# vmanam0451/distributed-path-tracer

Hardware: AMD Instinct MI355X
Metric: Msamples/sec, Cornell box 1920x1080, 256 spp per frame, 8 bounces (camera paths traced per second) (higher is better)
Workload: dtype f32

## Files before the change

### distributed-path-tracer_amd/__init__.py

```python
import atexit
import ctypes as C
import os
import re
import weakref

import numpy as np

_HERE = os.path.dirname(os.path.abspath(__file__))
LIB_PATH = os.environ.get("PTX_LIB") or os.path.join(_HERE, "libptx_hip.so")
HEADER_PATH = os.path.join(os.path.dirname(_HERE), "include", "ptx.h")

OK, ERR_INVALID, ERR_IO, ERR_PARSE, ERR_NO_CAMERA, ERR_NO_DEVICE, ERR_HIP, ERR_UNSUPPORTED = range(8)
NO_SUN_LIGHT = 0xFFFFFFFF

(ARR_MODEL_XFORM, ARR_MODEL_AABB, ARR_MODEL_SURF, ARR_SURF_RANGE, ARR_MESH_AABB, ARR_VERTICES, ARR_TRIANGLES,
 ARR_MATERIALS, ARR_KD_NODES, ARR_KD_REFS, ARR_CAMERA, ARR_SUN, ARR_MODEL_NAMES, ARR_TEXTURES, ARR_TEXELS, ARR_SURF_TEX, ARR_TEXELS_F32,
 ARR_LIGHT_TRIS, ARR_LIGHT_CDF, ARR_LIGHT_GEOM, ARR_TRI_ISECT, ARR_RES_NODES, ARR_RES_REFS, ARR_RES_TRIS, ARR_LDS_ROOT,
 ARR_RES_PLAN, ARR_ENV_ROW_CDF, ARR_ENV_CELL_CDF, ARR_PUNCTUAL, ARR_PUNCTUAL_CDF, ARR_LENS) = range(31)
LDS_LEAF_ORDER_BIT = 0x80000000


class PtxError(RuntimeError):
    def __init__(self, code, msg):
        super().__init__(f"ptx error {code}: {msg}")
        self.code = code


class WorkItem(C.Structure):
    _fields_ = [("mesh_name", C.c_char_p), ("primitives", C.POINTER(C.c_int32)), ("n_primitives", C.c_uint32)]


class LoadOpts(C.Structure):
    _fields_ = [("camera_index", C.c_uint32), ("sun_light_index", C.c_uint32), ("filter_primitives", C.c_uint32),
                ("n_work", C.c_uint32), ("work", C.POINTER(WorkItem))]


class WorkerEvent(C.Structure):
    _fields_ = [("num_workers", C.c_int32), ("n_work_meshes", C.c_uint32), ("worker_id", C.c_char * 64),
                ("scene_root", C.c_char * 256), ("scene_bucket", C.c_char * 128)]


class SceneDesc(C.Structure):
    _fields_ = [("n_models", C.c_uint32), ("model_xform", C.c_void_p), ("model_surf", C.c_void_p),
                ("n_surfaces", C.c_uint32), ("surf_range", C.c_void_p), ("vertices", C.c_void_p),
                ("triangles", C.c_void_p), ("materials", C.c_void_p), ("camera", C.c_void_p), ("sun", C.c_void_p)]


class Camera(C.Structure):
    _fields_ = [("origin", C.c_float * 3), ("basis", C.c_float * 9), ("yfov", C.c_float), ("lens_radius", C.c_float),
                ("focus_distance", C.c_float), ("blades", C.c_uint32), ("blade_rotation", C.c_float)]


# ... 416 lines not shown
                return -1

        fn = MASK_EXCHANGE_FN(thunk)
        n = int(mask.numel()) if hasattr(mask, "numel") else int(mask.size)
        _check(lib().ptx_ctx_set_mask_exchange(self.h, fn, None, _ptr(mask), n))
        self._mask_exchange = (fn, mask)

    def mask_exchange_stats(self):
        calls, ms = C.c_uint64(), C.c_double()
        _check(lib().ptx_ctx_get_mask_exchange_stats(self.h, C.byref(calls), C.byref(ms)))
        return {"calls": calls.value, "wall_ms": ms.value}

    def close(self):
        if getattr(self, "h", None):
            lib().ptx_ctx_destroy(self.h)
            self.h = None
            self._mask_exchange = None

    def __del__(self):
        try:
            self.close()
        except Exception:
            pass


_ARR_DTYPE = {ARR_MODEL_XFORM: (np.float32, 12), ARR_MODEL_AABB: (np.float32, 6), ARR_MODEL_SURF: (np.int32, 2),
              ARR_SURF_RANGE: (np.int32, 8), ARR_MESH_AABB: (np.float32, 6), ARR_VERTICES: (np.float32, 11),
              ARR_TRIANGLES: (np.uint32, 3), ARR_MATERIALS: (np.float32, 11), ARR_KD_NODES: (np.uint32, 2),
              ARR_KD_REFS: (np.uint32, 1), ARR_CAMERA: (np.float32, 1), ARR_SUN: (np.float32, 1),
              ARR_TEXTURES: (np.uint32, 4), ARR_TEXELS: (np.uint8, 1), ARR_SURF_TEX: (np.int32, 7), ARR_TEXELS_F32: (np.float32, 1),
              ARR_LIGHT_TRIS: (np.uint32, 2), ARR_LIGHT_CDF: (np.float32, 1), ARR_LIGHT_GEOM: (np.float32, 4),
              ARR_TRI_ISECT: (np.uint32, 12), ARR_RES_NODES: (np.uint32, 2), ARR_RES_REFS: (np.uint32, 1), ARR_RES_TRIS: (np.uint32, 12),
              ARR_LDS_ROOT: (np.uint32, 1), ARR_RES_PLAN: (np.uint32, 1), ARR_ENV_ROW_CDF: (np.float32, 1), ARR_ENV_CELL_CDF: (np.float32, 1),
              ARR_PUNCTUAL: (np.float32, 16), ARR_PUNCTUAL_CDF: (np.float32, 1), ARR_LENS: (np.float32, 2)}


class Scene:

    def __init__(self, handle, ctx):
        self.h = handle
        self.ctx = ctx
        _live.add(self)

    @classmethod
    def load_gltf(cls, ctx, path, camera_index=0, sun_light_index=0, work=None):
        h = C.c_void_p()
        opts = LoadOpts(camera_index, sun_light_index, 0, 0, None)
        keep = []
        if work is not None:
            items = (WorkItem * max(len(work), 1))()
            for k, (name, prims) in enumerate(work.items()):
                arr = (C.c_int32 * max(len(prims), 1))(*prims)
                keep.append(arr)
                items[k] = WorkItem(name.encode(), arr, len(prims))
            opts = LoadOpts(camera_index, sun_light_index, 1, len(work), items)
        _check(lib().ptx_scene_load_gltf(ctx.h if ctx else None, os.fsencode(path), C.byref(opts), C.byref(h)))
        return cls(h, ctx)

    @classmethod
    def load_event(cls, ctx, event_json, local_scene_root):
        h, cfg, ev = C.c_void_p(), RenderCfg(), WorkerEvent()
        _check(lib().ptx_worker_event_load(ctx.h if ctx else None, os.fsencode(event_json), os.fsencode(local_scene_root),
                                           C.byref(h), C.byref(cfg), C.byref(ev)))
        info = dict(num_workers=ev.num_workers, n_work_meshes=ev.n_work_meshes, worker_id=ev.worker_id.decode(),
                    scene_root=ev.scene_root.decode(), scene_bucket=ev.scene_bucket.decode())
        return cls(h, ctx), cfg, info

# ... 413 lines not shown
```

### distributed-path-tracer_amd/csrc/api_internal.hpp

```cpp
#pragma once
#include <hip/hip_runtime.h>

#include <algorithm>
#include <atomic>
#include <cstdint>
#include <cstdio>
#include <cstdlib>
#include <cstring>
#include <mutex>
#include <string>
#include <vector>

#include "../../include/ptx.h"
#include "kernels.hpp"

#pragma GCC visibility push(hidden)

using namespace ptx;

int set_err(int code, const std::string& m);
#define HIP_TRY(expr)                                                                                           \
	do {                                                                                                        \
		hipError_t e_ = (expr);                                                                                 \
		if (e_ != hipSuccess) return set_err(PTX_ERR_HIP, std::string(#expr) + ": " + hipGetErrorString(e_));   \
// ... 31 lines not shown
	DevBuf round_ws;
	DevBuf denoise;
	DevBuf adaptive, adaptive_state, adaptive_stage;
	hipEvent_t adaptive_ev[2] = {nullptr, nullptr};
	struct MaskExchange {
		ptx_mask_exchange_fn fn = nullptr;
		void* user = nullptr;
		uint8_t* mask = nullptr;
		size_t bytes = 0;
		uint64_t calls = 0;
		double wall_ms = 0;
	} mask_exchange;
	struct WfSet {
		DevBuf qent, pair_hit, seg, first, mask, ctl, spill, stream_buf, flow;
		uint32_t* flow_host = nullptr;
	} wf;
	std::vector<hipEvent_t> events;
	bool timing_on = false;
	std::vector<hipEvent_t> step_events;
	ptx_kernel_timing timing{};
	uint32_t list_key[9] = {0, 0, 0, 0, 0, 0, 0, 0, 0};
	uint32_t list_len = 0;
};

struct ptx_scene {
	ptx_ctx* ctx = nullptr;
	FlatScene host;
	DevBuf d_models, d_surfaces, d_materials, d_nodes, d_refs, d_tris, d_shade, d_tex, d_texels, d_lut, d_spaces, d_model_space, d_wf_order;
	DevBuf d_res_nodes, d_res_refs, d_res_tris, d_texels_f, d_hot;
	DevScene dev{};
	double lds_area_share = 0;
	double wf_pairs_per_ray = 0;
	bool leaf_ordered = true;
	int lds_leaf_order = -1;
	size_t lds_budget = 0;
	int mode = MODE_GLOBAL;
	size_t lds_bytes = 0;
	struct LightList {
		bool built = false, on_device = false;
		std::vector<uint32_t> tris;
		std::vector<float> cdf, geom;
		std::vector<int32_t> surf_first;
		float area = 0;
	} lights;
	std::mutex lights_mu;
	DevBuf d_light_tris, d_light_cdf, d_light_geom, d_light_first;
	struct EnvTable {
		bool built = false, on_device = false;
		uint32_t w = 0, h = 0;
		std::vector<float> row_cdf, cell_cdf;
	} env_table;
	DevBuf d_env_row, d_env_cell;
	struct Punctual {
		bool on_device = false;
		std::vector<float> recs, cdf;
	} punctual;
	DevBuf d_punctual, d_punctual_cdf;
	DevBuf d_lens;
};

const ptx_scene::LightList* build_lights(ptx_scene* sc);
const ptx_scene::EnvTable* build_env_table(ptx_scene* sc);
void srgb_thresholds(float thr[256]);
int adaptive_decide_locked(ptx_ctx* c, uint32_t w, uint32_t h, const float4* d_a, const float4* d_b, float threshold, uint8_t* d_done, uint32_t* d_pixels, uint32_t& n_active,
                           double* select_ms);
int adaptive_decide_sharded_locked(ptx_ctx* c, uint32_t w, uint32_t h, const AdaptiveShard& shard, bool mask_on_device, const float4* d_a, const float4* d_b, float threshold,
// ... 114 lines not shown
```

### distributed-path-tracer_amd/csrc/api_render.cpp

```cpp
#include <cmath>

#include "api_internal.hpp"

namespace {

int32_t max_surfaces_per_model(const ptx_scene* sc) {
	int32_t m = 0;
	for (const ModelRec& mr : sc->host.models) m = std::max(m, mr.n_surfaces);
	return m;
}

constexpr uint64_t kWfPoolPairs = 1024ull << 20;
constexpr uint64_t kWfBatchPairs = 256ull << 20;
constexpr uint32_t kWfFlowWords = 64, kWfFlowRays = 58 , kWfFlowPeak = 60, kWfFlowOverflow = 63, kWfMaxRound = 56;
bool wf_eligible(const ptx_scene* sc) {
	const size_t n_surf = sc->host.surfaces.size();
	if (n_surf == 0 || n_surf > (size_t)kWfMaxSurfaces) return false;
	if (sc->mode == MODE_LDS || !sc->dev.tri_isect) return false;
	return sc->leaf_ordered && sc->dev.geom_bytes <= 0xFFFFFFFFull;
}
int pipeline_choice(const ptx_scene* sc) {
	if (!wf_eligible(sc)) return 0;
	if (const char* e = getenv("PTX_WAVEFRONT")) return e[0] == '1' ? 1 : 0;
	if (getenv("PTX_FORCE_GLOBAL") || getenv("PTX_NO_HYBRID")) return 0;
// ... 223 lines not shown

int render_stats(ptx_ctx* c, const PassFrame& f, bool wavefront, const WfPlan& plan, const WfClock& clk, unsigned long long wf_rays, ptx_render_stats* stats) {
	unsigned long long rays = 0;
	HIP_TRY(hipMemcpy(&rays, (char*)c->counters.p + 16, 8, hipMemcpyDeviceToHost));
	if (const int rc = f.stats(c, rays + wf_rays, stats); rc != PTX_OK) return rc;
	const double ms = stats->kernel_ms;
	ptx_kernel_timing& tm = c->timing;
	tm.pipeline = wavefront ? 1u : 0u;
	tm.pool_pairs = wavefront ? plan.W.pool_cap : 0;
	tm.workspace_bytes = wavefront ? wf_workspace_bytes(c) : c->queues.cap + c->spill.cap;
	if (!wavefront) { tm.fused_ms = ms; tm.fused_launches = f.n_pass; }
	for (size_t k = 0; k + 4 <= clk.n_step_ev; k += 4) {
		float t0 = 0, t1 = 0, t2 = 0;
		HIP_TRY(hipEventElapsedTime(&t0, c->step_events[k], c->step_events[k + 1]));
		HIP_TRY(hipEventElapsedTime(&t1, c->step_events[k + 1], c->step_events[k + 2]));
		HIP_TRY(hipEventElapsedTime(&t2, c->step_events[k + 2], c->step_events[k + 3]));
		tm.classify_ms += t0; tm.traverse_ms += t1; tm.shade_ms += t2;
		tm.steps++;
	}
	tm.traverse_drain_frac = clk.all > 0 ? 1.0 - clk.busy / clk.all : 0.0;
#ifdef PTX_CLK
	if (!wavefront) {
		unsigned long long clks[8];
		HIP_TRY(hipMemcpy(clks, (char*)c->counters.p + 64, sizeof clks, hipMemcpyDeviceToHost));
		static const char* names[8] = {"kernel", "chunk_fetch", "extend_entry_loads", "extend_sweep_rest", "set_aside_lists", "shade_entry_hit_loads", "shade_hitrec_gathers", "shade_rest"};
		for (int k = 0; k < 8; k++) fprintf(stderr, "CLK %-22s %12llu kcycles summed over waves (%.2f %% of the waves' time)\n", names[k], clks[k], 100.0 * clks[k] / (double)clks[0]);
	}
#endif
#ifdef PTX_PROF
	unsigned long long prof[2 * kProfRegions];
	HIP_TRY(hipMemcpy(prof, (char*)c->counters.p + 64, sizeof prof, hipMemcpyDeviceToHost));
	static const char* names[kProfRegions] = {"extend_iter", "model_iter", "space_xform", "inline_model", "mesh_call", "mesh_pop", "node_step",
	                                           "tri_test", "defer_iter", "shade_iter", "defer_mesh_call", "defer_mesh_pop", "defer_node_step", "defer_tri_test",
	                                           "list_append", "shade_hit", "vertex_miss", "vertex_back_face", "vertex_last", "vertex_full"};
	for (int k = 0; k < kProfRegions; k++)
		fprintf(stderr, "PROF %-16s trips %12llu lanes %14llu  util %.3f  trips/64rays %.3f\n", names[k], prof[2 * k], prof[2 * k + 1],
		        prof[2 * k] ? (double)prof[2 * k + 1] / (64.0 * prof[2 * k]) : 0.0, (double)prof[2 * k] / ((double)rays / 64.0));
#endif
	return PTX_OK;
}

int render_frame_locked(ptx_scene* sc, const ptx_render_cfg* cfg, const char* who, float* accum, uint8_t* claimed, ptx_render_stats* stats, const PixelSubset* subset) {
	PassFrame f;
	f.cfg = cfg;
	if (const int rc = render_rect(cfg, who, true, f.x0, f.y0, f.w, f.h); rc != PTX_OK) return rc;
	ptx_ctx* c = sc->ctx;
	if (stats) *stats = ptx_render_stats{};
	if (const int rc = f.plan(c, sc, who, subset, 128ull << 20, 0xFFFFFFFFull); rc != PTX_OK || !f.n_pass) return rc;
	const uint32_t pass_spp = f.pass_spp, n_pass = f.n_pass;
	const uint64_t n_pixels = f.n_pixels;

	const int grid = c->n_cu;
	const size_t n_slots = (size_t)grid * (kBlock / 64);
	const uint32_t n_surf = (uint32_t)sc->host.surfaces.size(), n_mod = (uint32_t)sc->host.models.size();
	bool surface_units = max_surfaces_per_model(sc) >= 8 && n_surf <= (uint32_t)kMaxDeferModels;
	if (const char* e = getenv("PTX_SURFACE_UNITS")) surface_units = e[0] == '1' && n_surf <= (uint32_t)kMaxDeferModels;
	const uint32_t queue_stride = queue_float4_per_wave(surface_units ? n_surf : n_mod);
	bool wavefront = use_wavefront(sc);
	HIP_TRY(c->sample_rad.ensure((size_t)pass_spp * n_pixels * sizeof(float4)));
	HIP_TRY(c->counters.ensure(1024));
	HIP_TRY(c->spill.ensure(n_slots * (size_t)kSpillWords * sizeof(uint2)));
	unsigned long long* chunk_counter = (unsigned long long*)c->counters.p;
	unsigned long long* ray_counter = (unsigned long long*)((char*)c->counters.p + 16);
	HIP_TRY(hipMemsetAsync(c->counters.p, 0, 1024, c->stream));

	const bool dev_accum = is_device_ptr(accum);
	Staged s_accum, s_claimed;
// ... 756 lines not shown
```

### distributed-path-tracer_amd/csrc/device_core.hpp

```cpp
#pragma once
#include <hip/hip_runtime.h>
#include <stdint.h>
#include <stdlib.h>
#include <stdio.h>

#include "kernels.hpp"

namespace ptx {

#define DEV __device__ __forceinline__

#ifdef PTX_PROF
struct Prof { uint32_t t[kProfRegions], l[kProfRegions]; };
#define PROF_ARG , Prof& prof
#define PROF_PASS , prof
#define PROF(k) do { const uint64_t m_ = __ballot(true); prof.l[k] += 1u; prof.t[k] += ((threadIdx.x & 63u) == (uint32_t)(__ffsll((long long)m_) - 1)) ? 1u : 0u; } while (0)
#else
#define PROF_ARG
#define PROF_PASS
#define PROF(k) do { } while (0)
#endif

constexpr float kEps = 0.0001f;
constexpr double kPi = 3.14159265358979323846;
// ... 244 lines not shown
			else {
				if (sp < kRegStack + kSpillStack) {
					if (sp >= kRegStack) spill_put(spill, sp - kRegStack, n2, m2);
					n2 = n1; m2 = m1; n1 = n0; m1 = m0; n0 = has_second ? second : kNoNode; m0 = split_dist;
					sp++;
				}
				next = first; has_next = has_first;
				max_dist = split_dist;
			}
			if (!has_next) { valid = false; break; }
			node = next;
#ifdef PTX_LDS_PAIR_FETCH
			nd = pair_fetch ? (next == li ? kid0 : kid1) : g.nodes[node];
#else
			nd = (pair_fetch && g.pair) ? (next == li ? kid0 : kid1) : g.nodes[node];
#endif
		}
		if (!valid) continue;
		uint32_t first_ref = nd.x, count = nd.y >> 2;
		float best_t = -1.0f, bb1 = 0, bb2 = 0;
		uint32_t best_tri = 0;
		uint32_t key = 0;
		leaf_trip<true, PB>(g, first_ref, count, pr, max_dist, best_t, bb1, bb2, best_tri, key PROF_PASS);
		if (key >= kRcpKeyEnd) {
			best_t = -1.0f; bb1 = 0; bb2 = 0; best_tri = 0;
			leaf_trip<false, PB>(g, first_ref, count, pr, max_dist, best_t, bb1, bb2, best_tri, key PROF_PASS);
		}
		if (!(best_t >= 0)) continue;
		out.t = best_t; out.b1 = bb1; out.b2 = bb2; out.tri = best_tri;
		return true;
	}
}

DEV Geom lds_geom(const Geom& lds, uint32_t lds_root) { return {lds.nodes, lds.refs, lds.tris, (lds_root & kLdsLeafOrderBit) != 0, lds.pair}; }
template <int MODE, int PB>
DEV bool mesh_traverse_m(const Geoms& G, const SurfaceRec& sf, float nr, float fr, V3 o, V3 d, MeshHit& out, const Spill& spill PROF_ARG) {
	if constexpr (MODE == MODE_GLOBAL) return mesh_traverse<PB>(G.glb, sf.kd_root, nr, fr, o, d, out, spill PROF_PASS);
	else if constexpr (MODE == MODE_LDS) return mesh_traverse<PB>(lds_geom(G.lds, sf.lds_root), sf.lds_root & ~kLdsLeafOrderBit, nr, fr, o, d, out, spill PROF_PASS);
	else {
		if (sf.lds_root != 0xFFFFFFFFu) return mesh_traverse<PB>(lds_geom(G.lds, sf.lds_root), sf.lds_root & ~kLdsLeafOrderBit, nr, fr, o, d, out, spill PROF_PASS);
		return mesh_traverse<PB>(G.glb, sf.kd_root, nr, fr, o, d, out, spill PROF_PASS);
	}
}
template <int MODE, int PB>
DEV bool mesh_intersect_m(const Geoms& G, const SurfaceRec& sf, V3 o, V3 d, V3 inv, MeshHit& out, const Spill& spill PROF_ARG) {
	float nr, fr;
	if (!aabb_test_inv(sf.bmin, sf.bmax, o, inv, nr, fr)) return false;
	return mesh_traverse_m<MODE, PB>(G, sf, nr, fr, o, d, out, spill PROF_PASS);
}

struct SceneHit { float dist; int surface; uint32_t tri; float b1, b2; };

template <int MODE>
DEV bool scene_traverse(const DevScene& S, const Geoms& g, V3 o, V3 d, SceneHit& best, const Spill& spill) {
#ifdef PTX_PROF
	Prof prof{};
#endif
	best.dist = -1.0f;
	best.surface = -1;
	uint32_t cur_space = 0xFFFFFFFFu;
	V3 lo = o, ld = d, inv = d;
	for (int m = 0; m < S.n_models; m++) {
		const ModelRec& M = S.models[m];
		const uint32_t spc = S.model_space[m];
		if (spc != cur_space) {
			const SpaceRec& SP = S.spaces[spc];
			lo = mulmv(SP.inv_basis, o) + mk(SP.inv_origin[0], SP.inv_origin[1], SP.inv_origin[2]);
			ld = normalize(mulmv(SP.inv_basis, d));
			inv = mk(1.0f / ld.x, 1.0f / ld.y, 1.0f / ld.z);
			cur_space = spc;
		}
		float nr, fr;
		if (!aabb_test_inv(M.bmin, M.bmax, lo, inv, nr, fr)) continue;
// ... 570 lines not shown
```

### distributed-path-tracer_amd/csrc/flat_scene.hpp

```cpp
#pragma once
#include <cstdint>
#include <vector>
#include <string>

namespace ptx {

struct KdNode { uint32_t w0, w1; };
constexpr uint32_t KD_LEAF = 3u;
inline KdNode kd_make_branch(float split, uint32_t axis, bool has_l, bool has_r, uint32_t first_child) {
	uint32_t bits;
	__builtin_memcpy(&bits, &split, 4);
	return {bits, axis | (has_l ? 4u : 0u) | (has_r ? 8u : 0u) | (first_child << 4)};
}
inline KdNode kd_make_leaf(uint32_t first_ref, uint32_t count) { return {first_ref, KD_LEAF | (count << 2)}; }

struct TriRec { float ax, ay, az; uint32_t ia; float bx, by, bz; uint32_t ib; float cx, cy, cz; uint32_t ic; };

struct TriIsect { float e2y, e1z, e2z, e1y; float e1x, e2x, ay, az; float ax, c3, p0, p1; };
TriIsect make_tri_isect(const float* a, const float* b, const float* c, uint32_t gid);

struct HitRec { float a[3], ua, b[3], ub, c[3], uc, na[3], va, nb[3], vb, nc[3], vc, ta[3], p0, tb[3], p1, tc[3], p2; };
static_assert(sizeof(HitRec) == 144, "HitRec layout");

struct ModelRec {
	float inv_basis[9];
	float inv_origin[3];
	float basis[9];
	float origin[3];
	float nmat[9];
	float bmin[3], bmax[3];
	int32_t first_surface, n_surfaces;
	float pbmin[3], pbmax[3];
	float pad0;
	float box[6], pbox[6];
};
static_assert(sizeof(ModelRec) == 60 * 4, "ModelRec layout");

struct SurfaceRec {
	float bmin[3], bmax[3];
	uint32_t kd_root;
	uint32_t tri_base;
	uint32_t lds_root;
	uint32_t model;
	float pbmin[3], pbmax[3];
	float box[6], pbox[6];
};
static_assert(sizeof(SurfaceRec) == 28 * 4, "SurfaceRec layout");
constexpr uint32_t kLdsLeafOrderBit = 0x80000000u;
template <class Rec> inline void interleave_boxes(Rec& r) {
	for (int k = 0; k < 3; k++) { r.box[2 * k] = r.bmin[k]; r.box[2 * k + 1] = r.bmax[k]; r.pbox[2 * k] = r.pbmin[k]; r.pbox[2 * k + 1] = r.pbmax[k]; }
}

#ifdef __HIP__
#define PTX_HD __attribute__((host)) __attribute__((device))
#else
#define PTX_HD
#endif
struct RoughConsts { float r4, r4m1, smith_k; };
PTX_HD inline float pmax_hd(float a, float b) { return b > a ? b : a; }
PTX_HD inline float clamp_roughness(float roughness) { return pmax_hd(roughness, 0.05F); }
PTX_HD inline RoughConsts rough_consts(float roughness) {
	RoughConsts c;
	c.r4 = roughness * roughness;
	c.r4 *= c.r4;
	c.r4m1 = c.r4 - 1;
	const float r = roughness + 1;
	c.smith_k = (r * r) / 8;
	return c;
}
PTX_HD inline float fresnel_f0sq(float ior) {
	float f0 = (ior - 1) / (ior + 1);
	f0 *= f0;
	return f0;
}

struct MaterialRec {
	float albedo[3]; float opacity;
	float emissive[3]; float roughness;
	float metallic; float ior; uint32_t shadow_catcher; uint32_t tex_mask;
	int32_t tex[7];
	float f0sq;
// ... 38 lines not shown
	std::vector<TexRec> textures;
	std::vector<uint8_t> texels;
	std::vector<float> texels_f;
	std::vector<std::string> texture_paths;
	std::vector<ModelRec> models;
	std::vector<SurfaceRec> surfaces;
	std::vector<MaterialRec> materials;
	std::vector<ShadeRec> shade;
	std::vector<SpaceRec> spaces;
	std::vector<uint32_t> model_space;
	std::vector<KdNode> kd_nodes;
	std::vector<uint32_t> kd_refs;
	std::vector<TriRec> tris;
	std::vector<TriIsect> tri_isect;
	std::vector<HitRec> hitrec;
	std::vector<HitRec> hot_hitrec;
	CameraRec camera{};
	SunRec sun{};
	uint32_t kd_max_depth = 0;
	bool any_texture = false;
	bool any_alpha = false;
	int32_t env_tex = -1;

	std::vector<KdNode> res_nodes;
	std::vector<uint32_t> res_refs;
	std::vector<TriIsect> res_tris;
	uint32_t n_resident = 0;
	size_t res_bytes = 0;

	size_t geometry_bytes() const { return kd_nodes.size() * 8 + kd_refs.size() * 4 + tris.size() * 48; }
};

constexpr size_t kLdsLeafOrderCap = 4096;
void plan_residency(FlatScene& s, size_t lds_budget, bool lds_leaf_order = true);

void finalize_scene(FlatScene& s, const float* camera13, const float* sun13);
void apply_model_xforms(FlatScene& s);
std::vector<float> lens_table(const CameraRec& cam);

struct Error {
	int code;
	std::string msg;
};
void read_png(const std::string& path, uint32_t& W, uint32_t& H, uint32_t& C, std::vector<uint8_t>& out);
void read_jpeg(const std::string& path, uint32_t& W, uint32_t& H, uint32_t& C, std::vector<uint8_t>& out);
bool is_hdr_file(const std::string& path);
void read_hdr(const std::string& path, uint32_t& W, uint32_t& H, uint32_t& C, std::vector<float>& out);
void read_image(const std::string& path, uint32_t& W, uint32_t& H, uint32_t& C, std::vector<uint8_t>& out);
TexRec load_texture(FlatScene& s, const std::string& path, bool srgb);
struct WorkFilter {
	bool filter = false;
	std::vector<std::pair<std::string, std::vector<int32_t>>> work;
};
void load_gltf(const std::string& path, uint32_t camera_index, uint32_t sun_light_index, const WorkFilter& work, FlatScene& out);
void read_gltf_punctual_lights(const std::string& path, std::vector<float>& out);

struct WorkerEvent {
	WorkFilter work;
	std::string scene_bucket, scene_root, worker_id;
	int32_t num_workers = 1, samples = 0, bounces = 0;
	float X = 0, Y = 0;
};
void parse_worker_event(const std::string& json_path, WorkerEvent& out);

}
```

### distributed-path-tracer_amd/csrc/kernels.hpp

```cpp
#pragma once
#include <hip/hip_runtime.h>
#include <cstdint>
#include <cstdlib>

#include "flat_scene.hpp"

namespace ptx {

#ifndef PTX_BLOCK
#define PTX_BLOCK 1024
#endif
constexpr int kBlock = PTX_BLOCK;
#ifndef PTX_CHUNK
#define PTX_CHUNK 2048
#endif
constexpr uint32_t kChunk = PTX_CHUNK;
#ifndef PTX_INLINE_MIN
#define PTX_INLINE_MIN 32
#endif
constexpr uint32_t kInlineMin = PTX_INLINE_MIN;
constexpr uint32_t kListCap = (kChunk / 64u) * (kInlineMin - 1u) + 16u;
constexpr int kMaxDeferModels = 64;
constexpr uint32_t kQueueFixedFloat4 = 12u * kChunk + kChunk / 2u;
inline uint32_t queue_float4_per_wave(uint32_t n_units) { return kQueueFixedFloat4 + (n_units <= (uint32_t)kMaxDeferModels ? n_units : 0u) * 2u * kListCap; }
// ... 24 lines not shown
	const TexRec* tex;
	const uint8_t* texels;
	const float* texels_f;
	const float* srgb_lut;
	uint32_t glb_leaf_ordered;
	uint32_t any_texture;
	int32_t env_tex;
	const uint32_t* model_space;
	const uint32_t* wf_order;
	int32_t n_models;
	uint32_t n_surfaces, n_nodes, n_refs, n_tris;
	uint32_t any_alpha;
	uint32_t n_spaces;
	CameraRec cam;
	SunRec sun;
	const float2* lens;
};

struct RenderParams {
	uint32_t W, H;
	uint32_t x0, y0, w, h;
	uint32_t n_pixels;
	uint32_t sample0;
	uint32_t pass_spp;
	uint32_t bounces;
	uint32_t transparent;
	uint64_t n_paths;
	uint32_t seed_lo, seed_hi;
	float env[3];
	uint32_t integrator;
	const uint32_t* pixels;
};

constexpr int kProfRegions = 20;

struct PassBuffers {
	float4* queues;
	uint32_t queue_stride;
	uint32_t surface_units;
	float4* sample_rad;
	uint2* spill;
	unsigned long long* chunk_counter;
	unsigned long long* ray_counter;
};

struct IntersectArgs {
	const float *ox, *oy, *oz, *dx, *dy, *dz;
	size_t n;
	float* distance; int32_t* surface; int32_t* triangle;
	float *b0, *b1, *b2;
	float *px, *py, *pz, *nx, *ny, *nz, *u, *v;
	uint2* spill;
};

struct WfBuffers {
	float4* qent;
	float4* pair_hit;
	uint32_t pool_cap;
	uint2* seg;
	uint32_t seg_cap;
	uint32_t* first;
	unsigned long long* mask;
	uint32_t* ctl;
	const uint32_t* n_in;
	uint32_t* overflow;
	uint32_t* peak;
	uint2* spill;
// ... 171 lines not shown
```

### distributed-path-tracer_amd/csrc/ptx_api.cpp

```cpp
#include <cmath>

#include "api_internal.hpp"

namespace {
thread_local std::string g_err;
}
int set_err(int code, const std::string& m) { g_err = m; return code; }

void srgb_thresholds(float thr[256]) {
	auto byte_of = [](uint32_t bits) {
		float v;
		memcpy(&v, &bits, 4);
		return (uint32_t)(uint8_t)(std::pow(v, 1 / 2.2F) * 255 + 0.5F);
	};
	thr[0] = 0.0f;
	for (uint32_t k = 1; k < 256; k++) {
		uint32_t lo = 0, hi = 0x3F800000u;
		while (hi - lo > 1) {
			const uint32_t mid = lo + (hi - lo) / 2;
			if (byte_of(mid) >= k) hi = mid; else lo = mid;
		}
		memcpy(&thr[k], &hi, 4);
	}
}

namespace {

constexpr size_t kLdsBudget = 160 * 1024;
constexpr size_t kLeafOrderMaxBytes = (size_t)1 << 40;

void decide_mode(ptx_scene* sc) {
	FlatScene& h = sc->host;
	if (sc->lds_leaf_order < 0) {
		const char* e = getenv("PTX_LDS_LEAF_ORDER");
		sc->lds_leaf_order = (e && e[0] == '0') ? 0 : 1;
		sc->lds_budget = kLdsBudget;
		if (const char* b = getenv("PTX_LDS_BUDGET")) sc->lds_budget = std::min<size_t>(kLdsBudget, (size_t)strtoull(b, nullptr, 10));
	}
	plan_residency(h, sc->lds_budget, sc->lds_leaf_order != 0);
	if (getenv("PTX_FORCE_GLOBAL") || h.n_resident == 0) sc->mode = MODE_GLOBAL;
	else if (h.n_resident == h.surfaces.size()) sc->mode = MODE_LDS;
	else sc->mode = getenv("PTX_NO_HYBRID") ? MODE_GLOBAL : MODE_HYBRID;
	if (sc->mode == MODE_GLOBAL) for (auto& sr : h.surfaces) sr.lds_root = 0xFFFFFFFFu;
	sc->lds_bytes = sc->mode == MODE_GLOBAL ? 0 : h.res_bytes;
	{
		double all = 0, res = 0;
		for (const SurfaceRec& sr : h.surfaces) {
			const double ex = sr.bmax[0] - sr.bmin[0], ey = sr.bmax[1] - sr.bmin[1], ez = sr.bmax[2] - sr.bmin[2];
			const double a = (ex > 0 && ey > 0 && ez > 0) ? 2 * (ex * ey + ey * ez + ex * ez) : 0;
			all += a;
			if (sr.lds_root != 0xFFFFFFFFu) res += a;
		}
		sc->lds_area_share = all > 0 ? res / all : 0;
	}
	sc->leaf_ordered = h.kd_refs.size() * 48 <= kLeafOrderMaxBytes;
	if (const char* e = getenv("PTX_LEAF_ORDER")) sc->leaf_ordered = e[0] != '0';
}

int upload_scene(ptx_scene* sc) {
	ptx_ctx* c = sc->ctx;
	HIP_TRY(hipSetDevice(c->device));
	FlatScene& h = sc->host;
	auto up = [&](DevBuf& b, const void* src, size_t bytes, size_t padded) -> hipError_t {
		hipError_t e = b.ensure(std::max<size_t>(padded, 16));
		if (e != hipSuccess) return e;
		e = hipMemsetAsync(b.p, 0, std::max<size_t>(padded, 16), c->stream);
		if (e != hipSuccess) return e;
		return bytes ? hipMemcpyAsync(b.p, src, bytes, hipMemcpyHostToDevice, c->stream) : hipSuccess;
	};
	for (ModelRec& mr : h.models) interleave_boxes(mr);
	for (SurfaceRec& sr : h.surfaces) interleave_boxes(sr);
	HIP_TRY(up(sc->d_models, h.models.data(), h.models.size() * sizeof(ModelRec), h.models.size() * sizeof(ModelRec)));
// ... 652 lines not shown
		src = tmp.data(); bytes = tmp.size() * 4; break;
	case PTX_ARR_VERTICES: src = h.vertices.data(); bytes = h.vertices.size() * 4; break;
	case PTX_ARR_TRIANGLES: src = h.triangles.data(); bytes = h.triangles.size() * 4; break;
	case PTX_ARR_MATERIALS: src = h.materials_raw.data(); bytes = h.materials_raw.size() * 4; break;
	case PTX_ARR_KD_NODES: src = h.kd_nodes.data(); bytes = h.kd_nodes.size() * 8; break;
	case PTX_ARR_KD_REFS: src = h.kd_refs.data(); bytes = h.kd_refs.size() * 4; break;
	case PTX_ARR_CAMERA:
		tmp.assign(h.camera.origin, h.camera.origin + 3); tmp.insert(tmp.end(), h.camera.basis, h.camera.basis + 9);
		tmp.push_back(h.camera.fov); tmp.push_back(h.camera.tan_half_fov);
		src = tmp.data(); bytes = tmp.size() * 4; break;
	case PTX_ARR_SUN:
		if (h.sun.present) { tmp.assign(h.sun.basis, h.sun.basis + 9); tmp.insert(tmp.end(), h.sun.energy, h.sun.energy + 3); tmp.push_back(h.sun.angular_radius); }
		src = tmp.data(); bytes = tmp.size() * 4; break;
	case PTX_ARR_MODEL_NAMES:
		for (auto& n : h.model_names) names += n + "\n";
		src = names.data(); bytes = names.size(); elem = 1; break;
	case PTX_ARR_TEXTURES: src = h.textures.data(); bytes = h.textures.size() * sizeof(TexRec); break;
	case PTX_ARR_TEXELS: src = h.texels.data(); bytes = h.texels.size(); elem = 1; break;
	case PTX_ARR_SURF_TEX: src = h.surf_tex.data(); bytes = h.surf_tex.size() * 4; break;
	case PTX_ARR_TEXELS_F32: src = h.texels_f.data(); bytes = h.texels_f.size() * 4; break;
	case PTX_ARR_LIGHT_TRIS: { const auto& ll = *build_lights(const_cast<ptx_scene*>(sc)); src = ll.tris.data(); bytes = ll.tris.size() * 4; break; }
	case PTX_ARR_LIGHT_CDF: { const auto& ll = *build_lights(const_cast<ptx_scene*>(sc)); src = ll.cdf.data(); bytes = ll.cdf.size() * 4; break; }
	case PTX_ARR_LIGHT_GEOM: { const auto& ll = *build_lights(const_cast<ptx_scene*>(sc)); src = ll.geom.data(); bytes = ll.geom.size() * 4; break; }
	case PTX_ARR_ENV_ROW_CDF: { const auto& et = *build_env_table(const_cast<ptx_scene*>(sc)); src = et.row_cdf.data(); bytes = et.row_cdf.size() * 4; break; }
	case PTX_ARR_ENV_CELL_CDF: { const auto& et = *build_env_table(const_cast<ptx_scene*>(sc)); src = et.cell_cdf.data(); bytes = et.cell_cdf.size() * 4; break; }
	case PTX_ARR_PUNCTUAL: { std::lock_guard<std::mutex> tl(const_cast<ptx_scene*>(sc)->lights_mu); tmp = sc->punctual.recs; src = tmp.data(); bytes = tmp.size() * 4; break; }
	case PTX_ARR_PUNCTUAL_CDF: { std::lock_guard<std::mutex> tl(const_cast<ptx_scene*>(sc)->lights_mu); tmp = sc->punctual.cdf; src = tmp.data(); bytes = tmp.size() * 4; break; }
	case PTX_ARR_LENS: tmp = lens_table(h.camera); src = tmp.data(); bytes = tmp.size() * 4; break;
	case PTX_ARR_TRI_ISECT: src = h.tri_isect.data(); bytes = h.tri_isect.size() * sizeof(TriIsect); break;
	case PTX_ARR_RES_NODES: src = h.res_nodes.data(); bytes = h.res_nodes.size() * 8; break;
	case PTX_ARR_RES_REFS: src = h.res_refs.data(); bytes = h.res_refs.size() * 4; break;
	case PTX_ARR_RES_TRIS: src = h.res_tris.data(); bytes = h.res_tris.size() * sizeof(TriIsect); break;
	case PTX_ARR_LDS_ROOT:
		for (auto& s : h.surfaces) { float f; memcpy(&f, &s.lds_root, 4); tmp.push_back(f); }
		src = tmp.data(); bytes = tmp.size() * 4; break;
	case PTX_ARR_RES_PLAN: {
		const uint32_t w[4] = {(uint32_t)h.res_bytes, h.n_resident, (uint32_t)sc->lds_bytes, (uint32_t)h.hot_hitrec.size()};
		tmp.resize(4); memcpy(tmp.data(), w, 16);
		src = tmp.data(); bytes = 16; break;
	}
	default: set_err(PTX_ERR_INVALID, "unknown array id"); return -1;
	}
	if (dst) {
		if (dst_bytes < bytes) { set_err(PTX_ERR_INVALID, "destination too small"); return -1; }
		if (bytes) memcpy(dst, src, bytes);
	}
	return (int64_t)(bytes / elem);
}

}
```

### distributed-path-tracer_amd/csrc/scene_build.cpp

```cpp
#include "flat_scene.hpp"

#include <algorithm>
#include <cassert>
#include <cmath>
#include <cstdlib>
#include <cstring>
#include <deque>
#include <limits>
#include <atomic>
#include <exception>
#include <memory>
#include <mutex>
#include <thread>
#include <tuple>

namespace ptx {
namespace {

constexpr float kEps = 0.0001f;

struct F3 { float v[3]; };
struct Box { float lo[3], hi[3]; };

inline float pick_max(float a, float b) { return b > a ? b : a; }
// ... 345 lines not shown
		SpaceRec sp;
		memcpy(sp.inv_basis, s.models[mi].inv_basis, 36);
		memcpy(sp.inv_origin, s.models[mi].inv_origin, 12);
		size_t k = 0;
		for (; k < s.spaces.size(); k++) if (!memcmp(&s.spaces[k], &sp, sizeof sp)) break;
		if (k == s.spaces.size()) s.spaces.push_back(sp);
		s.model_space[mi] = (uint32_t)k;
	}
	s.shade.assign(n_surf, ShadeRec{});
	for (size_t mi = 0; mi < n_models; mi++)
		for (int32_t k = 0; k < s.models[mi].n_surfaces; k++) {
			ShadeRec& r = s.shade[s.models[mi].first_surface + k];
			memcpy(r.basis, s.models[mi].basis, 36);
			memcpy(r.origin, s.models[mi].origin, 12);
			memcpy(r.nmat, s.models[mi].nmat, 36);
			r.mat = s.materials[s.models[mi].first_surface + k];
			fill_shade_consts(r);
		}
}

std::vector<float> lens_table(const CameraRec& cam) {
	std::vector<float> t;
	if (!(cam.lens_radius > 0)) return t;
	const uint32_t n = cam.blades;
	for (uint32_t k = 0; k < n; k++) {
		const double th = (double)cam.blade_rotation + 2.0 * 3.14159265358979323846 * (double)k / (double)n;
		t.push_back((float)((double)cam.lens_radius * std::cos(th)));
		t.push_back((float)((double)cam.lens_radius * std::sin(th)));
	}
	t.push_back(t[0]); t.push_back(t[1]);
	return t;
}

void plan_residency(FlatScene& s, size_t lds_budget, bool lds_leaf_order) {
	const size_t n_surf = s.surfaces.size();
	s.res_nodes.clear(); s.res_refs.clear(); s.res_tris.clear();
	s.n_resident = 0;
	for (auto& sr : s.surfaces) sr.lds_root = 0xFFFFFFFFu;
	const size_t shade_bytes = s.shade.size() * sizeof(ShadeRec);
	auto bytes_of = [&](size_t si) {
		const int32_t* rg = &s.surf_range[8 * si];
		return (size_t)rg[5] * 8 + (size_t)rg[7] * 4 + (size_t)rg[3] * 48;
	};
	std::vector<size_t> order(n_surf);
	for (size_t i = 0; i < n_surf; i++) order[i] = i;
	std::stable_sort(order.begin(), order.end(), [&](size_t a, size_t b) { return bytes_of(a) < bytes_of(b); });
	std::vector<char> take(n_surf, 0);
	size_t used = shade_bytes + 48;
	for (size_t si : order) {
		if (used + bytes_of(si) > lds_budget) break;
		used += bytes_of(si);
		take[si] = 1;
	}
	std::vector<char> leaf_order(n_surf, 0);
	if (lds_leaf_order) {
		auto extra_of = [&](size_t si) {
			const int32_t* rg = &s.surf_range[8 * si];
			return ((int64_t)rg[7] - rg[3]) * 48 - (int64_t)rg[7] * 4;
		};
		std::vector<size_t> cand;
		for (size_t si = 0; si < n_surf; si++) if (take[si]) cand.push_back(si);
		std::stable_sort(cand.begin(), cand.end(), [&](size_t a, size_t b) { return extra_of(a) < extra_of(b); });
		const int64_t cap = (int64_t)std::min(kLdsLeafOrderCap, lds_budget > used ? lds_budget - used : (size_t)0);
		int64_t spent = 0;
		for (size_t si : cand) {
			const int64_t e = extra_of(si);
			if (e > 0) {
				if (spent + e > cap) break;
				spent += e;
			}
			leaf_order[si] = 1;
		}
	}
	for (size_t si = 0; si < n_surf; si++) {
		if (!take[si]) continue;
		const int32_t* rg = &s.surf_range[8 * si];
		const uint32_t t0 = (uint32_t)rg[2], nt = (uint32_t)rg[3], node0 = (uint32_t)rg[4], nn = (uint32_t)rg[5], ref0 = (uint32_t)rg[6], nr = (uint32_t)rg[7];
		const uint32_t nb = (uint32_t)s.res_nodes.size(), rb = (uint32_t)s.res_refs.size(), tb = (uint32_t)s.res_tris.size();
		for (uint32_t k = 0; k < nn; k++) {
			KdNode nd = s.kd_nodes[node0 + k];
			if ((nd.w1 & 3u) == KD_LEAF) nd.w0 = nd.w0 - ref0 + (leaf_order[si] ? tb : rb);
			else nd.w1 = (nd.w1 & 15u) | ((((nd.w1 >> 4) - node0) + nb) << 4);
			s.res_nodes.push_back(nd);
		}
		if (leaf_order[si]) {
			for (uint32_t k = 0; k < nr; k++) s.res_tris.push_back(s.tri_isect[s.kd_refs[ref0 + k]]);
		} else {
			for (uint32_t k = 0; k < nr; k++) s.res_refs.push_back(s.kd_refs[ref0 + k] - t0 + tb);
			for (uint32_t k = 0; k < nt; k++) s.res_tris.push_back(s.tri_isect[t0 + k]);
		}
		const uint32_t root = (s.surfaces[si].kd_root - node0) + nb;
		assert(root < kLdsLeafOrderBit);
		s.surfaces[si].lds_root = root | (leaf_order[si] ? kLdsLeafOrderBit : 0u);
		s.n_resident++;
	}
	s.res_bytes = s.res_tris.size() * 48 + shade_bytes + ((s.res_nodes.size() * 8 + 15) & ~(size_t)15) + ((s.res_refs.size() * 4 + 15) & ~(size_t)15);
}

}
```

### include/ptx.h

```cpp
#ifndef PTX_H
#define PTX_H

#include <stddef.h>
#include <stdint.h>

#ifdef __cplusplus
extern "C" {
#endif

typedef enum ptx_status {
	PTX_OK = 0,
	PTX_ERR_INVALID = 1,
	PTX_ERR_IO = 2,
	PTX_ERR_PARSE = 3,
	PTX_ERR_NO_CAMERA = 4,
	PTX_ERR_NO_DEVICE = 5,
	PTX_ERR_HIP = 6,
	PTX_ERR_UNSUPPORTED = 7
} ptx_status;

typedef struct ptx_ctx ptx_ctx;
typedef struct ptx_scene ptx_scene;

const char* ptx_last_error(void);
// ... 75 lines not shown
int ptx_scene_get_info(const ptx_scene* scene, ptx_scene_info* info);

typedef enum ptx_array {
	PTX_ARR_MODEL_XFORM = 0,
	PTX_ARR_MODEL_AABB = 1,
	PTX_ARR_MODEL_SURF = 2,
	PTX_ARR_SURF_RANGE = 3,
	PTX_ARR_MESH_AABB = 4,
	PTX_ARR_VERTICES = 5,
	PTX_ARR_TRIANGLES = 6,
	PTX_ARR_MATERIALS = 7,
	PTX_ARR_KD_NODES = 8,
	PTX_ARR_KD_REFS = 9,
	PTX_ARR_CAMERA = 10,
	PTX_ARR_SUN = 11,
	PTX_ARR_MODEL_NAMES = 12,
	PTX_ARR_TEXTURES = 13,
	PTX_ARR_TEXELS = 14,
	PTX_ARR_SURF_TEX = 15,
	PTX_ARR_TEXELS_F32 = 16,
	PTX_ARR_LIGHT_TRIS = 17,
	PTX_ARR_LIGHT_CDF = 18,
	PTX_ARR_LIGHT_GEOM = 19,
	PTX_ARR_TRI_ISECT = 20,
	PTX_ARR_RES_NODES = 21,
	PTX_ARR_RES_REFS = 22,
	PTX_ARR_RES_TRIS = 23,
	PTX_ARR_LDS_ROOT = 24,
	PTX_ARR_RES_PLAN = 25,
	PTX_ARR_ENV_ROW_CDF = 26,
	PTX_ARR_ENV_CELL_CDF = 27,
	PTX_ARR_PUNCTUAL = 28,
	PTX_ARR_PUNCTUAL_CDF = 29,
	PTX_ARR_LENS = 30
} ptx_array;
int64_t ptx_scene_get_array(const ptx_scene* scene, ptx_array which, void* dst, size_t dst_bytes);

typedef enum ptx_integrator { PTX_INTEGRATOR_LIB = 0, PTX_INTEGRATOR_WORKER = 1 } ptx_integrator;
typedef struct ptx_render_cfg {
	uint32_t W, H;
	uint32_t spp;
	uint32_t bounces;
	float env[3];
	uint32_t seed_lo, seed_hi;
	uint32_t x0, y0, w, h;
	uint32_t sample0;
	uint32_t spp_per_pass;
	uint32_t integrator;
	uint32_t shard_index, shard_count, shard_tile;
} ptx_render_cfg;
typedef struct ptx_render_stats {
	uint64_t rays;
	uint64_t samples;
	uint64_t passes;
	double kernel_ms;
} ptx_render_stats;
int ptx_render(ptx_scene* scene, const ptx_render_cfg* cfg, float* accum_rgba, ptx_render_stats* stats);

int ptx_render_transparent(ptx_scene* scene, const ptx_render_cfg* cfg, float* pixel_rgba, uint8_t* claimed, ptx_render_stats* stats);

typedef struct ptx_aov_buffers {
	float* albedo_cov;
	float* normal_depth;
} ptx_aov_buffers;
int ptx_render_aov(ptx_scene* scene, const ptx_render_cfg* cfg, const ptx_aov_buffers* out, ptx_render_stats* stats);

typedef struct ptx_motion_prev {
// ... 157 lines not shown
```

Baseline: 1640.

## Specialize LDS kd-tree traversal for leaf-only and shallow complete trees

Classifies each LDS-resident mesh kd-tree at build time as a single leaf or a shallow complete tree (at most three branch levels) and tags its root with shape bits. At traversal time, leaf-only meshes skip the traversal loop and test the leaf directly, and complete trees use a fixed three-entry register stack with no spill handling. The aim is less control flow and fewer registers for the small meshes in scenes like the Cornell box. In exchange it adds more code paths, which can raise register pressure and divergence in the megakernel.

```diff
diff --git a/distributed-path-tracer_amd/__init__.py b/distributed-path-tracer_amd/__init__.py
--- a/distributed-path-tracer_amd/__init__.py
+++ b/distributed-path-tracer_amd/__init__.py
@@ -16,8 +16,12 @@
 (ARR_MODEL_XFORM, ARR_MODEL_AABB, ARR_MODEL_SURF, ARR_SURF_RANGE, ARR_MESH_AABB, ARR_VERTICES, ARR_TRIANGLES,
  ARR_MATERIALS, ARR_KD_NODES, ARR_KD_REFS, ARR_CAMERA, ARR_SUN, ARR_MODEL_NAMES, ARR_TEXTURES, ARR_TEXELS, ARR_SURF_TEX, ARR_TEXELS_F32,
  ARR_LIGHT_TRIS, ARR_LIGHT_CDF, ARR_LIGHT_GEOM, ARR_TRI_ISECT, ARR_RES_NODES, ARR_RES_REFS, ARR_RES_TRIS, ARR_LDS_ROOT,
- ARR_RES_PLAN, ARR_ENV_ROW_CDF, ARR_ENV_CELL_CDF, ARR_PUNCTUAL, ARR_PUNCTUAL_CDF, ARR_LENS) = range(31)
+ ARR_RES_PLAN, ARR_ENV_ROW_CDF, ARR_ENV_CELL_CDF, ARR_PUNCTUAL, ARR_PUNCTUAL_CDF, ARR_LENS, ARR_LDS_SHAPE) = range(32)
 LDS_LEAF_ORDER_BIT = 0x80000000
+LDS_LEAF_ONLY_BIT = 0x40000000
+LDS_COMPLETE_BIT = 0x20000000
+LDS_ROOT_MASK = 0x1FFFFFFF
+KD_SHAPE_MAX_BRANCH_LEVELS = 3
 
 
 class PtxError(RuntimeError):
@@ -500,7 +504,8 @@
               ARR_LIGHT_TRIS: (np.uint32, 2), ARR_LIGHT_CDF: (np.float32, 1), ARR_LIGHT_GEOM: (np.float32, 4),
               ARR_TRI_ISECT: (np.uint32, 12), ARR_RES_NODES: (np.uint32, 2), ARR_RES_REFS: (np.uint32, 1), ARR_RES_TRIS: (np.uint32, 12),
               ARR_LDS_ROOT: (np.uint32, 1), ARR_RES_PLAN: (np.uint32, 1), ARR_ENV_ROW_CDF: (np.float32, 1), ARR_ENV_CELL_CDF: (np.float32, 1),
-              ARR_PUNCTUAL: (np.float32, 16), ARR_PUNCTUAL_CDF: (np.float32, 1), ARR_LENS: (np.float32, 2)}
+              ARR_PUNCTUAL: (np.float32, 16), ARR_PUNCTUAL_CDF: (np.float32, 1), ARR_LENS: (np.float32, 2),
+              ARR_LDS_SHAPE: (np.uint32, 1)}
 
 
 class Scene:
diff --git a/distributed-path-tracer_amd/csrc/api_internal.hpp b/distributed-path-tracer_amd/csrc/api_internal.hpp
--- a/distributed-path-tracer_amd/csrc/api_internal.hpp
+++ b/distributed-path-tracer_amd/csrc/api_internal.hpp
@@ -87,6 +87,7 @@
 	double lds_area_share = 0;
 	double wf_pairs_per_ray = 0;
 	bool leaf_ordered = true;
+	int kd_shapes = 1;
 	int lds_leaf_order = -1;
 	size_t lds_budget = 0;
 	int mode = MODE_GLOBAL;
diff --git a/distributed-path-tracer_amd/csrc/api_render.cpp b/distributed-path-tracer_amd/csrc/api_render.cpp
--- a/distributed-path-tracer_amd/csrc/api_render.cpp
+++ b/distributed-path-tracer_amd/csrc/api_render.cpp
@@ -279,7 +279,8 @@
 	HIP_TRY(hipMemcpy(prof, (char*)c->counters.p + 64, sizeof prof, hipMemcpyDeviceToHost));
 	static const char* names[kProfRegions] = {"extend_iter", "model_iter", "space_xform", "inline_model", "mesh_call", "mesh_pop", "node_step",
 	                                           "tri_test", "defer_iter", "shade_iter", "defer_mesh_call", "defer_mesh_pop", "defer_node_step", "defer_tri_test",
-	                                           "list_append", "shade_hit", "vertex_miss", "vertex_back_face", "vertex_last", "vertex_full"};
+	                                           "list_append", "shade_hit", "vertex_miss", "vertex_back_face", "vertex_last", "vertex_full",
+	                                           "leaf_only_call", "complete_pop", "complete_node_step", "defer_leaf_only_call", "defer_complete_pop", "defer_complete_node_step"};
 	for (int k = 0; k < kProfRegions; k++)
 		fprintf(stderr, "PROF %-16s trips %12llu lanes %14llu  util %.3f  trips/64rays %.3f\n", names[k], prof[2 * k], prof[2 * k + 1],
 		        prof[2 * k] ? (double)prof[2 * k + 1] / (64.0 * prof[2 * k]) : 0.0, (double)prof[2 * k] / ((double)rays / 64.0));
diff --git a/distributed-path-tracer_amd/csrc/device_core.hpp b/distributed-path-tracer_amd/csrc/device_core.hpp
--- a/distributed-path-tracer_amd/csrc/device_core.hpp
+++ b/distributed-path-tracer_amd/csrc/device_core.hpp
@@ -300,13 +300,92 @@
 	}
 }
 
+static_assert(kShapeMaxBranchLevels == kRegStack, "a complete tree's pending entries must fit the register stack");
+template <int PB> constexpr int shape_prof_base() { return PB == 4 ? 20 : 23; }
+template <int PB>
+DEV bool shape_leaf(const Geom& g, uint2 nd, const PRay& pr, float max_dist, MeshHit& out PROF_ARG) {
+	const uint32_t first_ref = nd.x, count = nd.y >> 2;
+	float best_t = -1.0f, bb1 = 0, bb2 = 0;
+	uint32_t best_tri = 0;
+	uint32_t key = 0;
+#ifdef PTX_PROF
+	for (uint32_t i = 0; i < count; i++) PROF(PB + 3);
+#endif
+	leaf_records<true, true>(g, first_ref, count, pr, max_dist, best_t, bb1, bb2, best_tri, key);
+	if (key >= kRcpKeyEnd) {
+		best_t = -1.0f; bb1 = 0; bb2 = 0; best_tri = 0;
+		leaf_records<false, true>(g, first_ref, count, pr, max_dist, best_t, bb1, bb2, best_tri, key);
+	}
+	if (!(best_t >= 0)) return false;
+	out.t = best_t; out.b1 = bb1; out.b2 = bb2; out.tri = best_tri;
+	return true;
+}
+template <int PB>
+DEV bool mesh_traverse_leaf(const Geom& g, uint32_t root, float fr, V3 o, V3 d, MeshHit& out PROF_ARG) {
+	PROF(shape_prof_base<PB>());
+	const PRay pr = pack_ray(o, d);
+	return shape_leaf<PB>(g, g.nodes[root], pr, fr, out PROF_PASS);
+}
+template <int PB>
+DEV bool mesh_traverse_complete(const Geom& g, uint32_t root, float nr, float fr, V3 o, V3 d, MeshHit& out PROF_ARG) {
+	PROF(PB);
+	const PRay pr = pack_ray(o, d);
+	int sp = 0;
+	uint32_t n0 = 0, n1 = 0, n2 = 0;
+	float m0 = 0, m1 = 0, m2 = 0;
+	uint32_t node = root;
+	float min_dist = nr, max_dist = fr;
+	for (;;) {
+		uint2 nd = g.nodes[node];
+		while ((nd.y & 3u) != KD_LEAF) {
+			PROF(shape_prof_base<PB>() + 2);
+			const uint32_t axis = nd.y & 3u;
+			const float split = __uint_as_float(nd.x);
+			const float oa = sel3(o, axis), da = sel3(d, axis);
+			const float split_dist = (split - oa) / da;
+			const uint32_t li = nd.y >> 4, ri = li + 1u;
+			const bool left_first = oa < split;
+			const uint32_t first = left_first ? li : ri, second = left_first ? ri : li;
+			uint32_t next;
+			if (split_dist < 0 || split_dist > max_dist) next = first;
+			else if (split_dist < min_dist) next = second;
+			else {
+				n2 = n1; m2 = m1; n1 = n0; m1 = m0; n0 = second; m0 = split_dist;
+				sp++;
+				next = first;
+				max_dist = split_dist;
+			}
+			node = next;
+			nd = g.nodes[node];
+		}
+		if (shape_leaf<PB>(g, nd, pr, max_dist, out PROF_PASS)) return true;
+		PROF(shape_prof_base<PB>() + 1);
+		if (sp == 0) return false;
+		sp--;
+		node = n0; min_dist = m0;
+		n0 = n1; m0 = m1; n1 = n2; m1 = m2;
+		max_dist = sp > 0 ? m0 : fr;
+	}
+}
+
 DEV Geom lds_geom(const Geom& lds, uint32_t lds_root) { return {lds.nodes, lds.refs, lds.tris, (lds_root & kLdsLeafOrderBit) != 0, lds.pair}; }
+template <int PB>
+DEV bool mesh_traverse_lds(const Geom& lds, uint32_t lds_root, float nr, float fr, V3 o, V3 d, MeshHit& out, const Spill& spill PROF_ARG) {
+	const uint32_t root = lds_root & kLdsRootMask;
+#ifndef PTX_NO_SHAPE_COMPLETE
+	if (lds_root & kLdsCompleteBit) return mesh_traverse_complete<PB>(lds, root, nr, fr, o, d, out PROF_PASS);
+#endif
+#ifndef PTX_NO_SHAPE_LEAF
+	if (lds_root & kLdsLeafOnlyBit) return mesh_traverse_leaf<PB>(lds, root, fr, o, d, out PROF_PASS);
+#endif
+	return mesh_traverse<PB>(lds_geom(lds, lds_root), root, nr, fr, o, d, out, spill PROF_PASS);
+}
 template <int MODE, int PB>
 DEV bool mesh_traverse_m(const Geoms& G, const SurfaceRec& sf, float nr, float fr, V3 o, V3 d, MeshHit& out, const Spill& spill PROF_ARG) {
 	if constexpr (MODE == MODE_GLOBAL) return mesh_traverse<PB>(G.glb, sf.kd_root, nr, fr, o, d, out, spill PROF_PASS);
-	else if constexpr (MODE == MODE_LDS) return mesh_traverse<PB>(lds_geom(G.lds, sf.lds_root), sf.lds_root & ~kLdsLeafOrderBit, nr, fr, o, d, out, spill PROF_PASS);
+	else if constexpr (MODE == MODE_LDS) return mesh_traverse_lds<PB>(G.lds, sf.lds_root, nr, fr, o, d, out, spill PROF_PASS);
 	else {
-		if (sf.lds_root != 0xFFFFFFFFu) return mesh_traverse<PB>(lds_geom(G.lds, sf.lds_root), sf.lds_root & ~kLdsLeafOrderBit, nr, fr, o, d, out, spill PROF_PASS);
+		if (sf.lds_root != 0xFFFFFFFFu) return mesh_traverse_lds<PB>(G.lds, sf.lds_root, nr, fr, o, d, out, spill PROF_PASS);
 		return mesh_traverse<PB>(G.glb, sf.kd_root, nr, fr, o, d, out, spill PROF_PASS);
 	}
 }
diff --git a/distributed-path-tracer_amd/csrc/flat_scene.hpp b/distributed-path-tracer_amd/csrc/flat_scene.hpp
--- a/distributed-path-tracer_amd/csrc/flat_scene.hpp
+++ b/distributed-path-tracer_amd/csrc/flat_scene.hpp
@@ -47,6 +47,10 @@
 };
 static_assert(sizeof(SurfaceRec) == 28 * 4, "SurfaceRec layout");
 constexpr uint32_t kLdsLeafOrderBit = 0x80000000u;
+constexpr uint32_t kLdsLeafOnlyBit = 0x40000000u;
+constexpr uint32_t kLdsCompleteBit = 0x20000000u;
+constexpr uint32_t kLdsRootMask = 0x1FFFFFFFu;
+constexpr int kShapeMaxBranchLevels = 3;
 template <class Rec> inline void interleave_boxes(Rec& r) {
 	for (int k = 0; k < 3; k++) { r.box[2 * k] = r.bmin[k]; r.box[2 * k + 1] = r.bmax[k]; r.pbox[2 * k] = r.pbmin[k]; r.pbox[2 * k + 1] = r.pbmax[k]; }
 }
@@ -151,7 +155,8 @@
 };
 
 constexpr size_t kLdsLeafOrderCap = 4096;
-void plan_residency(FlatScene& s, size_t lds_budget, bool lds_leaf_order = true);
+void plan_residency(FlatScene& s, size_t lds_budget, bool lds_leaf_order = true, bool kd_shapes = true);
+uint32_t kd_tree_shape(const std::vector<KdNode>& nodes, uint32_t root);
 
 void finalize_scene(FlatScene& s, const float* camera13, const float* sun13);
 void apply_model_xforms(FlatScene& s);
diff --git a/distributed-path-tracer_amd/csrc/kernels.hpp b/distributed-path-tracer_amd/csrc/kernels.hpp
--- a/distributed-path-tracer_amd/csrc/kernels.hpp
+++ b/distributed-path-tracer_amd/csrc/kernels.hpp
@@ -80,7 +80,7 @@
 	const uint32_t* pixels;
 };
 
-constexpr int kProfRegions = 20;
+constexpr int kProfRegions = 26;
 
 struct PassBuffers {
 	float4* queues;
diff --git a/distributed-path-tracer_amd/csrc/ptx_api.cpp b/distributed-path-tracer_amd/csrc/ptx_api.cpp
--- a/distributed-path-tracer_amd/csrc/ptx_api.cpp
+++ b/distributed-path-tracer_amd/csrc/ptx_api.cpp
@@ -34,10 +34,12 @@
 	if (sc->lds_leaf_order < 0) {
 		const char* e = getenv("PTX_LDS_LEAF_ORDER");
 		sc->lds_leaf_order = (e && e[0] == '0') ? 0 : 1;
+		const char* k = getenv("PTX_KD_SHAPES");
+		sc->kd_shapes = (k && k[0] == '0') ? 0 : 1;
 		sc->lds_budget = kLdsBudget;
 		if (const char* b = getenv("PTX_LDS_BUDGET")) sc->lds_budget = std::min<size_t>(kLdsBudget, (size_t)strtoull(b, nullptr, 10));
 	}
-	plan_residency(h, sc->lds_budget, sc->lds_leaf_order != 0);
+	plan_residency(h, sc->lds_budget, sc->lds_leaf_order != 0, sc->kd_shapes != 0);
 	if (getenv("PTX_FORCE_GLOBAL") || h.n_resident == 0) sc->mode = MODE_GLOBAL;
 	else if (h.n_resident == h.surfaces.size()) sc->mode = MODE_LDS;
 	else sc->mode = getenv("PTX_NO_HYBRID") ? MODE_GLOBAL : MODE_HYBRID;
@@ -756,7 +758,11 @@
 	case PTX_ARR_RES_REFS: src = h.res_refs.data(); bytes = h.res_refs.size() * 4; break;
 	case PTX_ARR_RES_TRIS: src = h.res_tris.data(); bytes = h.res_tris.size() * sizeof(TriIsect); break;
 	case PTX_ARR_LDS_ROOT:
-		for (auto& s : h.surfaces) { float f; memcpy(&f, &s.lds_root, 4); tmp.push_back(f); }
+	case PTX_ARR_LDS_SHAPE:
+		for (auto& s : h.surfaces) {
+			const uint32_t w = (which == PTX_ARR_LDS_SHAPE || s.lds_root == 0xFFFFFFFFu) ? s.lds_root : (s.lds_root & (kLdsRootMask | kLdsLeafOrderBit));
+			float f; memcpy(&f, &w, 4); tmp.push_back(f);
+		}
 		src = tmp.data(); bytes = tmp.size() * 4; break;
 	case PTX_ARR_RES_PLAN: {
 		const uint32_t w[4] = {(uint32_t)h.res_bytes, h.n_resident, (uint32_t)sc->lds_bytes, (uint32_t)h.hot_hitrec.size()};
diff --git a/distributed-path-tracer_amd/csrc/scene_build.cpp b/distributed-path-tracer_amd/csrc/scene_build.cpp
--- a/distributed-path-tracer_amd/csrc/scene_build.cpp
+++ b/distributed-path-tracer_amd/csrc/scene_build.cpp
@@ -401,7 +401,24 @@
 	return t;
 }
 
-void plan_residency(FlatScene& s, size_t lds_budget, bool lds_leaf_order) {
+uint32_t kd_tree_shape(const std::vector<KdNode>& nodes, uint32_t root) {
+	if (root >= nodes.size()) return 0u;
+	if ((nodes[root].w1 & 3u) == KD_LEAF) return kLdsLeafOnlyBit;
+	std::vector<std::pair<uint32_t, int>> todo{{root, 0}};
+	while (!todo.empty()) {
+		const auto [n, above] = todo.back();
+		todo.pop_back();
+		if (n >= nodes.size()) return 0u;
+		const uint32_t w1 = nodes[n].w1;
+		if ((w1 & 3u) == KD_LEAF) continue;
+		if ((w1 & 12u) != 12u || above + 1 > kShapeMaxBranchLevels) return 0u;
+		todo.push_back({w1 >> 4, above + 1});
+		todo.push_back({(w1 >> 4) + 1u, above + 1});
+	}
+	return kLdsCompleteBit;
+}
+
+void plan_residency(FlatScene& s, size_t lds_budget, bool lds_leaf_order, bool kd_shapes) {
 	const size_t n_surf = s.surfaces.size();
 	s.res_nodes.clear(); s.res_refs.clear(); s.res_tris.clear();
 	s.n_resident = 0;
@@ -459,8 +476,9 @@
 			for (uint32_t k = 0; k < nt; k++) s.res_tris.push_back(s.tri_isect[t0 + k]);
 		}
 		const uint32_t root = (s.surfaces[si].kd_root - node0) + nb;
-		assert(root < kLdsLeafOrderBit);
-		s.surfaces[si].lds_root = root | (leaf_order[si] ? kLdsLeafOrderBit : 0u);
+		assert(root <= kLdsRootMask);
+		const uint32_t shape = (kd_shapes && leaf_order[si]) ? kd_tree_shape(s.res_nodes, root) : 0u;
+		s.surfaces[si].lds_root = root | (leaf_order[si] ? kLdsLeafOrderBit : 0u) | shape;
 		s.n_resident++;
 	}
 	s.res_bytes = s.res_tris.size() * 48 + shade_bytes + ((s.res_nodes.size() * 8 + 15) & ~(size_t)15) + ((s.res_refs.size() * 4 + 15) & ~(size_t)15);
diff --git a/include/ptx.h b/include/ptx.h
--- a/include/ptx.h
+++ b/include/ptx.h
@@ -131,7 +131,8 @@
 	PTX_ARR_ENV_CELL_CDF = 27,
 	PTX_ARR_PUNCTUAL = 28,
 	PTX_ARR_PUNCTUAL_CDF = 29,
-	PTX_ARR_LENS = 30
+	PTX_ARR_LENS = 30,
+	PTX_ARR_LDS_SHAPE = 31
 } ptx_array;
 int64_t ptx_scene_get_array(const ptx_scene* scene, ptx_array which, void* dst, size_t dst_bytes);
 
```

New measurement: 1707, median of 6. +4.1%, better.
